# wusize/CLIPSelf

Hardware: AMD Instinct MI355X
Metric: images/sec (student+teacher distill step), ViT-B/16 32 crops/img (higher is better)
Workload: dtype bf16; 1 GPU; EVA02-CLIP-B-16 CLIPSelf image-patches step, 64 images x 32 crops per GPU, 224^2 (BASELINE configs[1]); global_batch=64, crops_per_image=32, image_size=224, parallelism=dp1, teacher_chunk=2048, teacher_last_block=cls_query_only, teacher_schedule=one_batch_ahead_on_side_stream

## Files before the change

clipself_amd/csrc/gemm_stream.hip:

```cpp
#include <vector>
#include <cstdio>
#include "gemm_common.h"

namespace {

typedef __attribute__((ext_vector_type(2))) unsigned u32x2;
typedef __attribute__((ext_vector_type(4))) unsigned u32x4;

constexpr unsigned OOB = 0xfffffff0u;

__device__ __forceinline__ float lane_bcast(int src_lane_x4, float v) {
    return __int_as_float(__builtin_amdgcn_ds_bpermute(src_lane_x4, __float_as_int(v)));
}
__device__ __forceinline__ unsigned pack2(float a, float b) {
    union { bf16x2 v; unsigned u; } pk;
    pk.v[0] = f2bf(a);
    pk.v[1] = f2bf(b);
    return pk.u;
}
__device__ __forceinline__ void swap32(unsigned& x, unsigned& y) {
    const u32x2 r = __builtin_amdgcn_permlane32_swap(x, y, false, false);
    x = r[0];
    y = r[1];
}
// ... 356 lines not shown

template <bool LN, bool AUX, int CP>
__device__ __forceinline__ void epi_swiglu_slab(const GemmArgs& p, const f32x16 (&acc)[4][2], int lane, int row0, int tn, int wn, const EpiOps& eo,
                                                char* slab) {
    const int l31 = lane & 31, hf = lane >> 5;
    const int hbase = tn * 128 + wn * 32;
    const bool colok = hbase < p.group;
    float nm[4], rs[4];
#pragma unroll
    for (int i = 0; i < 4; ++i) {
        rs[i] = LN ? eo.rstd[i] : 1.f;
        nm[i] = LN ? -eo.rstd[i] * eo.mean[i] : 0.f;
    }
    float ssum[4] = {0.f, 0.f, 0.f, 0.f}, ssq[4] = {0.f, 0.f, 0.f, 0.f};
    const int sl0 = hf << 4;
#pragma unroll
    for (int q = 0; q < 4; ++q) {
        float hv[4][4];
#pragma unroll
        for (int r = 0; r < 4; ++r) {
            const int e = q * 4 + r;
            const int sl = sl0 + ((8 * q + r) << 2);
            const float b1 = lane_bcast(sl, eo.cb), b2 = lane_bcast(sl + 128, eo.cb);
            float c1 = 0.f, c2 = 0.f;
            if (LN) { c1 = lane_bcast(sl, eo.cc); c2 = lane_bcast(sl + 128, eo.cc); }
#pragma unroll
            for (int i = 0; i < 4; ++i) {
                float u = acc[i][0][e], v = acc[i][1][e];
                if (LN) {
                    u = fmaf(rs[i], u, fmaf(nm[i], c1, b1));
                    v = fmaf(rs[i], v, fmaf(nm[i], c2, b2));
                } else {
                    u += b1;
                    v += b2;
                }
                hv[i][r] = silu_mul(u, v);
            }
        }
#pragma unroll
        for (int i = 0; i < 4; ++i) {
            const unsigned d0 = pack2(hv[i][0], hv[i][1]), d1 = pack2(hv[i][2], hv[i][3]);
            if (AUX) {
                ssum[i] = dot2_bf16(d1, 0x3f803f80u, dot2_bf16(d0, 0x3f803f80u, ssum[i]));
                ssq[i] = dot2_bf16(d1, d1, dot2_bf16(d0, d0, ssq[i]));
            }
            const int lrow = i * 32 + l31;
            const int s8 = (2 * q + hf) ^ (((lrow >> 1) & 3) << 1);
            *(uint2*)(slab + lrow * 64 + s8 * 8) = make_uint2(d0, d1);
        }
    }
    const __amdgpu_buffer_rsrc_t rc = make_rsrc((const __bf16*)p.C + (size_t)row0 * p.ldc + hbase);
    const int piece = lane & 3;
#pragma unroll
    for (int k = 0; k < 8; ++k) {
        const int lrow = (lane >> 2) + 16 * k;
        const uint4 w = *(const uint4*)(slab + lrow * 64 + ((piece ^ ((lrow >> 1) & 3)) << 4));
        const bool ok = colok && row0 + lrow < p.M && !CS_ABL(p, 8);
        store16<CP>(u32x4{w.x, w.y, w.z, w.w}, rc, ok ? (unsigned)(lrow * p.ldc + piece * 8) * 2u : OOB);
    }
    if (AUX) {
        const size_t slice = (size_t)tn * 4 + wn;
        const __amdgpu_buffer_rsrc_t rst = make_rsrc(p.stats_part + (slice * p.M + row0) * 2);
#pragma unroll
        for (int i = 0; i < 4; ++i) {
            const float s = both_halves(ssum[i]), q2 = both_halves(ssq[i]);
            const bool ok = colok && hf == 0 && row0 + i * 32 + l31 < p.M && !CS_ABL(p, 8);
            store8<CP>(u32x2{__float_as_uint(s), __float_as_uint(q2)}, rst, ok ? (unsigned)(i * 32 + l31) * 8u : OOB);
        }
    }
}

#ifdef CS_ABLATION_SWITCHES
__device__ unsigned long long* g_epi_trace = nullptr;
#define EPI_TRACE(slot)                                                                                                            \
    do {                                                                                                                           \
        if (g_epi_trace && (threadIdx.x & 63) == 0)                                                                                \
            g_epi_trace[((size_t)blockIdx.x * 8 + (threadIdx.x >> 6)) * 16 + (slot)] = __builtin_amdgcn_s_memrealtime();           \
    } while (0)
#define EPI_TRACE_WAIT() do { if (g_epi_trace) asm volatile("s_waitcnt vmcnt(0)" ::: "memory"); } while (0)
#else
#define EPI_TRACE(slot) do { } while (0)
#define EPI_TRACE_WAIT() do { } while (0)
#endif
template <bool LN, bool AUX, int CP, bool F8 = false, int SPLIT = 0, int FM = 4>
__device__ __forceinline__ void epi_resid_slab(const GemmArgs& p, const f32x16 (&acc)[FM][2], int lane, int row0, int colw, int tn, int wn,
                                               const EpiOps& eo, char* slab) {
    static_assert(!(SPLIT & 2) || AUX, "a split stream leaves together with the row statistics");
    const int l31 = lane & 31, hf = lane >> 5;
    const int rrow = lane >> 3, piece = lane & 7, col = colw + piece * 8;
    const bool colok = col < p.N;
    const __amdgpu_buffer_rsrc_t rc = make_rsrc((SPLIT & 2) ? (const void*)p.xb_out : (const void*)((const float*)p.C + (size_t)row0 * p.ldc + colw));
    const __amdgpu_buffer_rsrc_t rx = make_rsrc((SPLIT & 1) ? (const void*)p.xb_out : (const void*)(p.extra + (size_t)row0 * p.ldc + colw));
    const __amdgpu_buffer_rsrc_t rb = make_rsrc((AUX || SPLIT) ? (const void*)(p.xb_out + (size_t)row0 * p.ldxb + colw) : (const void*)p.C);
    const __amdgpu_buffer_rsrc_t rl = make_rsrc(SPLIT ? (const void*)(p.lo + (size_t)row0 * p.ldxb + colw) : (const void*)p.A);
    const size_t slice = (size_t)tn * 4 + wn;
    const __amdgpu_buffer_rsrc_t rst = make_rsrc(AUX ? (const void*)(p.stats_part + (slice * p.M + row0) * 2) : (const void*)p.C);
    f32x4 cb4[2] = {{0.f, 0.f, 0.f, 0.f}, {0.f, 0.f, 0.f, 0.f}}, cc4[2] = {{0.f, 0.f, 0.f, 0.f}, {0.f, 0.f, 0.f, 0.f}};
#pragma unroll
    for (int h = 0; h < 2; ++h) {
        const unsigned off = colok ? (unsigned)(col + 4 * h) * 4u : OOB;
        if (p.bias) cb4[h] = __builtin_bit_cast(f32x4, __builtin_amdgcn_raw_buffer_load_b128(make_rsrc(p.bias), off, 0, 0));
        if (LN || F8) cc4[h] = __builtin_bit_cast(f32x4, __builtin_amdgcn_raw_buffer_load_b128(make_rsrc(p.ln_colsum), off, 0, 0));
    }
    EPI_TRACE(0);
#pragma unroll
    for (int i = 0; i < FM; ++i) {
        f32x4 xin[4][2];
#pragma unroll
        for (int it = 0; it < 4; ++it) {
            const int rrel = i * 32 + rrow + 8 * it;
            const bool ok = colok && row0 + rrel < p.M;
            if constexpr (SPLIT & 1) {
                const unsigned off = ok ? (unsigned)(rrel * p.ldxb + piece * 8) * 2u : OOB;
                const u32x4 h = __builtin_bit_cast(u32x4, __builtin_amdgcn_raw_buffer_load_b128(rb, off, 0, CP));
                const u32x4 l = __builtin_bit_cast(u32x4, __builtin_amdgcn_raw_buffer_load_b128(rl, off, 0, CP));
#pragma unroll
                for (int w = 0; w < 4; ++w) {
                    xin[it][w >> 1][2 * (w & 1)] = __uint_as_float(__builtin_amdgcn_perm(h[w], l[w], 0x05040100u) - 0x8000u);
                    xin[it][w >> 1][2 * (w & 1) + 1] = __uint_as_float(__builtin_amdgcn_perm(h[w], l[w], 0x07060302u) - 0x8000u);
                }
            } else {
                const unsigned off = ok ? (unsigned)(rrel * p.ldc + piece * 8) * 4u : OOB;
                xin[it][0] = __builtin_bit_cast(f32x4, __builtin_amdgcn_raw_buffer_load_b128(rx, off, 0, CP));
                xin[it][1] = __builtin_bit_cast(f32x4, __builtin_amdgcn_raw_buffer_load_b128(rx, ok ? off + 16u : OOB, 0, CP));
            }
        }
        const float rs_row = (LN || F8) ? eo.rstd[i] : 1.f, nm_row = LN ? -eo.rstd[i] * eo.mean[i] : 0.f;
#pragma unroll
        for (int j = 0; j < 2; ++j)
#pragma unroll
            for (int q = 0; q < 4; ++q) {
                f32x4 t;
#pragma unroll
                for (int r = 0; r < 4; ++r) t[r] = acc[i][j][q * 4 + r];
                const int s16 = (j * 8 + 2 * q + hf) ^ (l31 & 15);
                *(f32x4*)(slab + l31 * 256 + s16 * 16) = t;
            }
        EPI_TRACE(1 + 3 * i);
        EPI_TRACE_WAIT();
        EPI_TRACE(2 + 3 * i);
        const int sel = lane & 7;
        float st_s = 0.f, st_q = 0.f;
#pragma unroll
        for (int it = 0; it < 4; ++it) {
            const int lrow = rrow + 8 * it, rrel = i * 32 + lrow;
            const bool ok = colok && row0 + rrel < p.M;
            float rs = 1.f, nm = 0.f;
            if (LN || F8) rs = lane_bcast(lrow << 2, rs_row);
            if (LN) nm = lane_bcast(lrow << 2, nm_row);
            f32x4 o[2];
#pragma unroll
            for (int h = 0; h < 2; ++h) {
                const f32x4 sv = *(const f32x4*)(slab + lrow * 256 + (((2 * piece + h) ^ (lrow & 15)) << 4));
                if (LN) {
#pragma unroll
                    for (int t = 0; t < 4; ++t) o[h][t] = xin[it][h][t] + fmaf(rs, sv[t], fmaf(nm, cc4[h][t], cb4[h][t]));
                } else if (F8) {
#pragma unroll
                    for (int t = 0; t < 4; ++t) o[h][t] = xin[it][h][t] + fmaf(rs * cc4[h][t], sv[t], cb4[h][t]);
                } else {
                    o[h] = xin[it][h] + (sv + cb4[h]);
                }
            }
            if constexpr (SPLIT & 2) {
                const unsigned off = ok ? (unsigned)(rrel * p.ldxb + piece * 8) * 2u : OOB;
                unsigned y[8];
#pragma unroll
                for (int t = 0; t < 8; ++t) y[t] = __float_as_uint(o[t >> 2][t & 3]) + 0x8000u;
                store16<CP>(u32x4{__builtin_amdgcn_perm(y[1], y[0], 0x07060302u), __builtin_amdgcn_perm(y[3], y[2], 0x07060302u),
                                  __builtin_amdgcn_perm(y[5], y[4], 0x07060302u), __builtin_amdgcn_perm(y[7], y[6], 0x07060302u)}, rb, off);
                store16<CP>(u32x4{__builtin_amdgcn_perm(y[1], y[0], 0x05040100u), __builtin_amdgcn_perm(y[3], y[2], 0x05040100u),
                                  __builtin_amdgcn_perm(y[5], y[4], 0x05040100u), __builtin_amdgcn_perm(y[7], y[6], 0x05040100u)}, rl, off);
            } else {
                const unsigned off = ok ? (unsigned)(rrel * p.ldc + piece * 8) * 4u : OOB;
                store16<CP>(__builtin_bit_cast(u32x4, o[0]), rc, off);
                store16<CP>(__builtin_bit_cast(u32x4, o[1]), rc, ok ? off + 16u : OOB);
            }
            if (AUX) {
                if constexpr (!(SPLIT & 2))
                    store16<CP>(u32x4{pack2(o[0][0], o[0][1]), pack2(o[0][2], o[0][3]), pack2(o[1][0], o[1][1]), pack2(o[1][2], o[1][3])}, rb,
                                ok ? (unsigned)(rrel * p.ldxb + piece * 8) * 2u : OOB);
                float ps = 0.f, pq = 0.f;
                if (colok) {
#pragma unroll
                    for (int t = 0; t < 8; ++t) { ps += o[t >> 2][t & 3]; pq = fmaf(o[t >> 2][t & 3], o[t >> 2][t & 3], pq); }
                }
                const float a = sum_lanes8(ps), b = sum_lanes8(pq);
                if (sel == it) { st_s = a; st_q = b; }
            }
        }
        if (AUX) {
            const int rrel = i * 32 + rrow + 8 * sel;
            const bool ok = sel < 4 && row0 + rrel < p.M && colw < p.N;
            store8<CP>(u32x2{__float_as_uint(st_s), __float_as_uint(st_q)}, rst, ok ? (unsigned)rrel * 8u : OOB);
        }
        EPI_TRACE(3 + 3 * i);
        __builtin_amdgcn_sched_barrier(0);
    }
}

template <int EPI, bool AUX, bool SLAB, int SPLIT = 0, int FM = 4, int MF = 32>
constexpr int epi_stores() {
    if (EPI == EPI_SWIGLU_BF16 && MF == 16) return 8 + (AUX ? 2 : 0);
    if (EPI == EPI_SWIGLU_BF16) return FM * (2 + (AUX ? 1 : 0));
    if (EPI == EPI_RESID_F32) return FM * (8 + (AUX ? ((SPLIT & 2) ? 0 : 4) + 1 : 0));
    return FM * 4;
}

#ifndef CS_DMA_AUX_A
#define CS_DMA_AUX_A 0
#endif
#ifndef CS_DMA_AUX_B
#define CS_DMA_AUX_B 0
#endif
#define CS_VMCNT(N) asm volatile("s_waitcnt vmcnt(%0)" ::"n"(N) : "memory")

inline bool getenv_flag(const char* name) {
    const char* v = getenv(name);
    return v && v[0] && v[0] != '0';
}

template <int EPI, bool LN, bool AUX, bool SLAB, bool F8 = false, int SPLIT = 0, int BMT = 256, int MF = 32>
__global__ __launch_bounds__(512) void gemm_stream_kernel(GemmArgs p) {
    static_assert(MF == 32 || (MF == 16 && LN && !SLAB && !F8 && SPLIT == 0 && BMT == 256 && (epi_is_bf16(EPI) ? !AUX : EPI == EPI_SWIGLU_BF16)),
                  "16x16x32 loop: the folded-LN bf16 and SwiGLU register epilogues");
    constexpr bool M16 = MF == 16;
    static_assert(BMT == 256 || (BMT == 192 && !F8 && SPLIT == 0 && !LN && !AUX), "192-row tiles: the training schedule's plain epilogues");
    static_assert(SPLIT == 0 || (EPI == EPI_RESID_F32 && LN && !F8), "the split stream belongs to the folded-LayerNorm residual epilogue");
    static_assert(SLAB || EPI != EPI_RESID_F32, "the fp32 residual epilogue exists in the slab form only (whole-line traffic)");
    static_assert(!F8 || (!LN && !AUX && (EPI == EPI_BF16 || EPI == EPI_RESID_F32)), "fp8 operands: bf16 and fp32-residual outputs");
    constexpr int ES = F8 ? 1 : 2;
    constexpr int CP = 0;
    constexpr bool SWI = EPI == EPI_SWIGLU_BF16, RES = EPI == EPI_RESID_F32;
    static_assert(SWI || RES || epi_is_bf16(EPI), "register epilogues");
    constexpr int BM = BMT, BN = 256, WN = 4, TM = BM / 2, TN = 64, FM = TM / 32, FN = 2;
    constexpr int A_BYTES = BM * BK * 2, B_BYTES = BN * BK * 2;
    constexpr int NPA = BM / 32;
    constexpr int NM = FM * FN, NR = FM + FN;
    constexpr int S = epi_stores<EPI, AUX, SLAB, SPLIT, FM, MF>() < 55 ? epi_stores<EPI, AUX, SLAB, SPLIT, FM, MF>() : 55;
    extern __shared__ __attribute__((aligned(16))) char smem[];
    const int tid = threadIdx.x, lane = tid & 63;
    const int wave = __builtin_amdgcn_readfirstlane(tid >> 6);
    const int wm = wave / WN, wn = wave - wm * WN;
    const int hf = M16 ? lane >> 4 : lane >> 5, l31 = M16 ? lane & 15 : lane & 31;
    char* const b_ring = smem + 3 * A_BYTES;
    const int ntiles = p.tiles_m * p.tiles_n, ktiles = p.K / (F8 ? 128 : BK);
    const int a_base = ((wm * TM + l31) >> 1) << 8, b_base = ((wn * TN + l31) >> 1) << 8;
    const int par8 = (l31 & 1) << 3, sw = l31 >> 1;
    const int G = gridDim.x;
#ifndef CS_NO_DMA_ROLES
    constexpr bool ROLES = !F8;
#else
    constexpr bool ROLES = false;
#endif
    const bool role_a = ROLES && wave >= 4;
#ifndef CS_NO_MID_BARRIER
    constexpr bool MID = ROLES && !SLAB && !F8;
#else
    constexpr bool MID = false;
#endif

    unsigned avoff[ROLES ? 8 : 4], bvoff[ROLES ? 1 : 4];
    const char *a_src = nullptr, *b_src = nullptr;
    int a_tile = blockIdx.x, a_kt = 0, b_tile = blockIdx.x, b_kt = 0;
    auto set_a = [&](int tile) {
        int tm, tn;
        tile_of_id(p, tile, ntiles, tm, tn);
        a_src = (const char*)p.A + (size_t)tm * BM * p.lda * ES;
#pragma unroll
        for (int i = 0; i < (ROLES ? NPA : 4); ++i) {
            int tr, chk;
            lane_source(ROLES ? (wave & 3) * NPA + i : wave * 4 + i, lane, tr, chk);
            avoff[i] = (unsigned)(min(tr, p.M - 1 - tm * BM) * p.lda * ES + chk * 16);
        }
    };
    auto set_b = [&](int tile) {
        int tm, tn;
        tile_of_id(p, tile, ntiles, tm, tn);
        if (SWI) {
            b_src = (const char*)p.B + (size_t)tn * (BN / 2) * p.ldb * ES;
        } else {
            b_src = (const char*)p.B + (size_t)tn * BN * p.ldb * ES;
        }
#pragma unroll
        for (int i = 0; i < (ROLES ? 8 : 4); ++i) {
            int tr, chk;
            lane_source(ROLES ? (wave & 3) * 8 + i : wave * 4 + i, lane, tr, chk);
            int rel;
            if (SWI) {
                const int hrel = (tr >> 6) * 32 + (tr & 31);
                rel = ((tr >> 5) & 1) * p.group + min(hrel, p.group - 1 - tn * (BN / 2));
            } else {
                rel = min(tr, p.N - 1 - tn * BN);
            }
            (ROLES ? avoff : bvoff)[i] = (unsigned)(rel * p.ldb * ES + chk * 16);
        }
    };
    auto adv_a = [&]() {
        if (++a_kt == ktiles) {
            a_kt = 0;
            if (a_tile + G < ntiles) {
                a_tile += G;
                set_a(a_tile);
            }
        }
    };
    auto adv_b = [&]() {
        if (++b_kt == ktiles) {
            b_kt = 0;
            if (b_tile + G < ntiles) {
                b_tile += G;
                set_b(b_tile);
            }
        }
    };
#define ISSUE_A(X, SLOT)                                                                                                      \
    __builtin_amdgcn_global_load_lds((const __attribute__((address_space(1))) void*)(a_src + (size_t)a_kt * (BK * 2) + avoff[X]), \
                                     (__attribute__((address_space(3))) void*)(smem + (SLOT) * A_BYTES + (wave * 4 + (X)) * 1024), 16, 0, CS_DMA_AUX_A)
#define ISSUE_B(X, SLOT)                                                                                                      \
    __builtin_amdgcn_global_load_lds((const __attribute__((address_space(1))) void*)(b_src + (size_t)b_kt * (BK * 2) + bvoff[X]), \
                                     (__attribute__((address_space(3))) void*)(b_ring + (SLOT) * B_BYTES + (wave * 4 + (X)) * 1024), 16, 0, CS_DMA_AUX_B)

#define ISSUE_RA(X, SLOT)                                                                                                     \
    __builtin_amdgcn_global_load_lds((const __attribute__((address_space(1))) void*)(a_src + (size_t)a_kt * (BK * 2) + avoff[X]), \
                                     (__attribute__((address_space(3))) void*)(smem + (SLOT) * A_BYTES + ((wave & 3) * NPA + (X)) * 1024), 16, 0, CS_DMA_AUX_A)
#define ISSUE_RB(X, SLOT)                                                                                                     \
    __builtin_amdgcn_global_load_lds((const __attribute__((address_space(1))) void*)(b_src + (size_t)b_kt * (BK * 2) + avoff[X]), \
                                     (__attribute__((address_space(3))) void*)(b_ring + (SLOT) * B_BYTES + ((wave & 3) * 8 + (X)) * 1024), 16, 0, CS_DMA_AUX_B)

    if constexpr (ROLES) {
        if (role_a) {
            set_a(a_tile);
#pragma unroll
            for (int x = 0; x < NPA; ++x) ISSUE_RA(x, 0);
            adv_a();
#pragma unroll
            for (int x = 0; x < NPA; ++x) ISSUE_RA(x, 1);
            adv_a();
        } else {
            set_b(b_tile);
#pragma unroll
            for (int x = 0; x < 8; ++x) ISSUE_RB(x, 0);
            adv_b();
            if constexpr (MID) {
#pragma unroll
                for (int x = 0; x < 8; ++x) ISSUE_RB(x, 1);
                adv_b();
            }
        }
        if constexpr (MID) {
            if (role_a) CS_VMCNT(NPA);
            else CS_VMCNT(8);
            __builtin_amdgcn_s_barrier();
        }
    } else {
        set_a(a_tile);
        set_b(b_tile);
#pragma unroll
        for (int x = 0; x < 4; ++x) ISSUE_A(x, 0);
        adv_a();
#pragma unroll
        for (int x = 0; x < 4; ++x) ISSUE_B(x, 0);
        adv_b();
#pragma unroll
        for (int x = 0; x < 4; ++x) ISSUE_A(x, 1);
        adv_a();
    }

    int curA = 0, gpar = 0;
    bool after_epi = false;
    for (int tile = blockIdx.x; tile < ntiles; tile += G) {
        int tm, tn;
        tile_of_id(p, tile, ntiles, tm, tn);
        const int row0 = tm * BM + wm * TM, colw = tn * BN + wn * TN;
        f32x16 acc[M16 ? 1 : FM][M16 ? 1 : FN];
        f32x4 acc16[M16 ? 8 : 1][M16 ? 4 : 1];
        constexpr int RB = M16 ? 16 : 32, NRB = TM / RB;
        EpiOpsT<M16 ? 8 : 4> eo;
        auto load_epi_ops = [&](int ln) {
            const int l31 = ln & (RB - 1), hf = ln >> 5, lane = ln;
#pragma unroll
            for (int i = 0; i < (M16 ? 8 : 4); ++i) eo.mean[i] = eo.rstd[i] = 0.f;
            eo.cb = eo.cc = 0.f;
            if (LN || F8) {
#pragma unroll
                for (int i = 0; i < NRB; ++i) {
                    const int r = min(row0 + i * RB + l31, p.M - 1);
                    if (LN) eo.mean[i] = p.ln_mean[r];
                    eo.rstd[i] = p.ln_rstd[r];
                }
            }
            int co;
            if (SWI) co = hf * p.group + min(tn * 128 + wn * 32 + (lane & 31), p.group - 1);
            else co = min(colw + lane, p.N - 1);
            if (!RES) {
                if (p.bias) eo.cb = p.bias[co];
                if (LN || F8) eo.cc = p.ln_colsum[co];
            }
        };

        auto ktile = [&](auto zero_tag, auto role_tag) {
            constexpr bool ZERO = decltype(zero_tag)::value;
            constexpr int ROLE = decltype(role_tag)::value;
            constexpr int KEEP = ROLE == 0 ? 4 : ROLE == 1 ? 0 : NPA;
            constexpr int SS = S + KEEP > 63 ? 63 - KEEP : S;
            if (after_epi) CS_VMCNT(KEEP + SS);
            else CS_VMCNT(KEEP);
            after_epi = false;
            asm volatile("s_waitcnt lgkmcnt(0)" ::: "memory");
            if (!CS_ABL(p, 2))
                __builtin_amdgcn_s_barrier();
            const char* la = smem + curA * A_BYTES + a_base;
            const char* lb = b_ring + gpar * B_BYTES + b_base;
            const int slot_a2 = curA == 0 ? 2 : curA - 1, slot_b1 = gpar ^ 1;
            if constexpr (F8) {
                typedef __attribute__((ext_vector_type(8))) int i32x8;
                typedef __attribute__((ext_vector_type(4))) int i32x4;
#pragma unroll
                for (int s2 = 0; s2 < 2; ++s2) {
                    const int c0 = 4 * s2 + 2 * hf;
                    const int off0 = ((par8 | c0) ^ sw) << 4, off1 = ((par8 | (c0 + 1)) ^ sw) << 4;
                    i32x8 a8[FM], b8[FN];
#pragma unroll
                    for (int i = 0; i < FM; ++i) {
                        const i32x4 lo = *(const i32x4*)(la + i * (16 * 256) + off0), hi = *(const i32x4*)(la + i * (16 * 256) + off1);
                        a8[i] = i32x8{lo[0], lo[1], lo[2], lo[3], hi[0], hi[1], hi[2], hi[3]};
                    }
#pragma unroll
                    for (int j = 0; j < FN; ++j) {
                        const i32x4 lo = *(const i32x4*)(lb + j * (16 * 256) + off0), hi = *(const i32x4*)(lb + j * (16 * 256) + off1);
                        b8[j] = i32x8{lo[0], lo[1], lo[2], lo[3], hi[0], hi[1], hi[2], hi[3]};
                    }
                    if constexpr (ROLE == 1) {
                        if (s2 == 0) {
#pragma unroll
                            for (int x = 0; x < 8; ++x) ISSUE_RB(x, slot_b1);
                        }
                    } else if constexpr (ROLE == 2) {
                        if (s2 == 1) {
#pragma unroll
                            for (int x = 0; x < NPA; ++x) ISSUE_RA(x, slot_a2);
                        }
                    } else if (s2 == 0) {
                        ISSUE_B(0, slot_b1); ISSUE_B(1, slot_b1); ISSUE_B(2, slot_b1); ISSUE_B(3, slot_b1);
                    } else {
                        ISSUE_A(0, slot_a2); ISSUE_A(1, slot_a2); ISSUE_A(2, slot_a2); ISSUE_A(3, slot_a2);
                    }
#pragma unroll
                    for (int i = 0; i < FM; ++i)
#pragma unroll
                        for (int j = 0; j < FN; ++j) {
                            if (ZERO && s2 == 0) {
                                const f32x16 z = {0.f, 0.f, 0.f, 0.f, 0.f, 0.f, 0.f, 0.f, 0.f, 0.f, 0.f, 0.f, 0.f, 0.f, 0.f, 0.f};
                                acc[i][j] = __builtin_amdgcn_mfma_scale_f32_32x32x64_f8f6f4(b8[j], a8[i], z, 0, 0, 0, 0x7f7f7f7f, 0, 0x7f7f7f7f);
                            } else {
                                acc[i][j] = __builtin_amdgcn_mfma_scale_f32_32x32x64_f8f6f4(b8[j], a8[i], acc[i][j], 0, 0, 0, 0x7f7f7f7f, 0, 0x7f7f7f7f);
                            }
                        }
                }
            } else {
                bf16x8 a[2][FM], b[2][FN];
                auto frags = [&](int ks, int buf) {
                    const int off = ((par8 | (ks * 2 + hf)) ^ sw) << 4;
#pragma unroll
                    for (int i = 0; i < FM; ++i) a[buf][i] = *(const bf16x8*)(la + i * (16 * 256) + off);
// ... 168 lines not shown
            };
            auto read_a = [&](const char* pa, int ks, int c) {
#pragma unroll
                for (int x = 0; x < 4; ++x) ga[c][x] = frag(pa, ks, c * 4 + x);
            };
            auto read_b = [&](const char* pb, int ks, int jj) {
                gb[2 * jj] = frag(pb, ks, 2 * jj);
                gb[2 * jj + 1] = frag(pb, ks, 2 * jj + 1);
            };
            auto mfmas = [&](int c, int jj, bool zero) {
#pragma unroll
                for (int x = 0; x < 4; ++x)
#pragma unroll
                    for (int j = 2 * jj; j < 2 * jj + 2; ++j) {
                        if (zero) {
                            const f32x4 z = {0.f, 0.f, 0.f, 0.f};
                            acc16[c * 4 + x][j] = __builtin_amdgcn_mfma_f32_16x16x32_bf16(gb[j], ga[c][x], z, 0, 0, 0);
                        } else {
                            acc16[c * 4 + x][j] = __builtin_amdgcn_mfma_f32_16x16x32_bf16(gb[j], ga[c][x], acc16[c * 4 + x][j], 0, 0, 0);
                        }
                    }
            };
            auto order = [&](auto r0a, auto nra, auto r0b, auto nrb, auto d0a, auto nda, auto d0b, auto ndb) {
#pragma unroll
                for (int m = 0; m < 16; ++m) {
                    __builtin_amdgcn_sched_group_barrier(0x008, 1, 0);
                    if ((m >= r0a.value && m < r0a.value + nra.value) || (m >= r0b.value && m < r0b.value + nrb.value))
                        __builtin_amdgcn_sched_group_barrier(0x100, 1, 0);
                    if ((m >= d0a.value && m < d0a.value + nda.value) || (m >= d0b.value && m < d0b.value + ndb.value))
                        __builtin_amdgcn_sched_group_barrier(0x010, 1, 0);
                }
            };
#define CI(N) std::integral_constant<int, (N)>{}
            if (ZERO) {
                read_a(la, 0, 0);
                read_b(lb, 0, 0);
                __builtin_amdgcn_sched_group_barrier(0x100, 6, 0);
            }
            read_b(lb, 0, 1);
            mfmas(0, 0, ZERO);
            read_a(la, 0, 1);
            mfmas(0, 1, ZERO);
            order(CI(0), CI(2), CI(8), CI(4), CI(0), CI(0), CI(0), CI(0));
            read_a(la, 1, 0);
            mfmas(1, 0, ZERO);
            read_b(lb, 1, 0);
            if constexpr (ROLE == 2) {
#pragma unroll
                for (int x = 0; x < NPA / 2; ++x) ISSUE_RA(x, slot_a2);
            }
            mfmas(1, 1, ZERO);
            order(CI(0), CI(4), CI(8), CI(2), CI(10), CI(ROLE == 2 ? NPA / 2 : 0), CI(0), CI(0));
            read_b(lb, 1, 1);
            if constexpr (ROLE == 2) {
#pragma unroll
                for (int x = NPA / 2; x < NPA; ++x) ISSUE_RA(x, slot_a2);
            }
            mfmas(0, 0, false);
            read_a(la, 1, 1);
            mfmas(0, 1, false);
            order(CI(0), CI(2), CI(8), CI(4), CI(2), CI(ROLE == 2 ? NPA / 2 : 0), CI(0), CI(0));
            {
                constexpr int KEEP = ROLE == 1 ? 0 : NPA;
                constexpr int SS = S + KEEP > 63 ? 63 - KEEP : S;
                if (after_epi) CS_VMCNT(KEEP + SS);
                else CS_VMCNT(KEEP);
                after_epi = false;
                asm volatile("s_waitcnt lgkmcnt(0)" ::: "memory");
                __builtin_amdgcn_s_barrier();
            }
            read_a(la_n, 0, 0);
            if constexpr (ROLE == 1) { ISSUE_RB(0, slot_b2); ISSUE_RB(1, slot_b2); ISSUE_RB(2, slot_b2); ISSUE_RB(3, slot_b2); }
            mfmas(1, 0, false);
            read_b(lb_n, 0, 0);
            if constexpr (ROLE == 1) { ISSUE_RB(4, slot_b2); ISSUE_RB(5, slot_b2); ISSUE_RB(6, slot_b2); ISSUE_RB(7, slot_b2); }
            mfmas(1, 1, false);
            order(CI(0), CI(4), CI(8), CI(2), CI(4), CI(ROLE == 1 ? 4 : 0), CI(10), CI(ROLE == 1 ? 4 : 0));
#undef CI
            if (ROLE == 1) adv_b();
            else adv_a();
            curA = nextA;
            gpar ^= 1;
        };
        if constexpr (M16) {
            if (role_a) {
                ktile_m16(std::true_type{}, std::integral_constant<int, 2>{});
                for (int kt = 1; kt < ktiles; ++kt) ktile_m16(std::false_type{}, std::integral_constant<int, 2>{});
            } else {
                ktile_m16(std::true_type{}, std::integral_constant<int, 1>{});
                for (int kt = 1; kt < ktiles; ++kt) ktile_m16(std::false_type{}, std::integral_constant<int, 1>{});
            }
        } else if constexpr (MID) {
            if (role_a) {
                ktile_mid(std::true_type{}, std::integral_constant<int, 2>{});
                for (int kt = 1; kt < ktiles; ++kt) ktile_mid(std::false_type{}, std::integral_constant<int, 2>{});
            } else {
                ktile_mid(std::true_type{}, std::integral_constant<int, 1>{});
                for (int kt = 1; kt < ktiles; ++kt) ktile_mid(std::false_type{}, std::integral_constant<int, 1>{});
            }
        } else if constexpr (ROLES) {
            if (role_a) {
                ktile(std::true_type{}, std::integral_constant<int, 2>{});
                for (int kt = 1; kt < ktiles; ++kt) ktile(std::false_type{}, std::integral_constant<int, 2>{});
            } else {
                ktile(std::true_type{}, std::integral_constant<int, 1>{});
                for (int kt = 1; kt < ktiles; ++kt) ktile(std::false_type{}, std::integral_constant<int, 1>{});
            }
        } else {
            ktile(std::true_type{}, std::integral_constant<int, 0>{});
            for (int kt = 1; kt < ktiles; ++kt) ktile(std::false_type{}, std::integral_constant<int, 0>{});
        }
        if (CS_ABL(p, 4)) continue;
        after_epi = true;
        int lane_e = lane;
        asm volatile("" : "+v"(lane_e));
        if constexpr (SLAB) {
            asm volatile("s_waitcnt lgkmcnt(0)" ::: "memory");
            __builtin_amdgcn_s_barrier();
            char* const slab = wave >= 4 ? b_ring + (gpar ^ 1) * B_BYTES + (wave - 4) * 8192
                               : (BM == 192 && wave == 3) ? b_ring + 2 * B_BYTES
                                                          : smem + (curA == 0 ? 2 : curA - 1) * A_BYTES + wave * 8192;
            load_epi_ops(lane_e);
#ifndef CS_NO_KERNARG_RELOAD
            constexpr bool RELOAD = RES && LN && AUX;
#else
            constexpr bool RELOAD = false;
#endif
            if constexpr (RELOAD) {
                const __attribute__((address_space(4))) GemmArgs* pk = (const __attribute__((address_space(4))) GemmArgs*)__builtin_amdgcn_kernarg_segment_ptr();
                asm volatile("" : "+s"(pk));
                GemmArgs pe;
                pe.A = pk->A; pe.C = pk->C; pe.bias = pk->bias; pe.extra = pk->extra; pe.M = pk->M; pe.N = pk->N; pe.ldc = pk->ldc;
                pe.ln_colsum = pk->ln_colsum; pe.stats_part = pk->stats_part; pe.xb_out = pk->xb_out; pe.ldxb = pk->ldxb; pe.lo = pk->lo;
                pe.dbg = pk->dbg;
                epi_resid_slab<LN, AUX, CP, F8, SPLIT, FM>(pe, acc, lane_e, row0, colw, tn, wn, eo, slab);
            } else if constexpr (RES) {
                epi_resid_slab<LN, AUX, CP, F8, SPLIT, FM>(p, acc, lane_e, row0, colw, tn, wn, eo, slab);
            } else {
                static_assert(FM == 4, "the slab forms of the bf16 / SwiGLU epilogues exist for 256-row tiles");
                if constexpr (SWI) epi_swiglu_slab<LN, AUX, CP>(p, acc, lane_e, row0, tn, wn, eo, slab);
                else epi_bf16_slab<epi_act(EPI), LN, CP>(p, acc, lane_e, row0, colw, eo, slab);
            }
        } else {
            load_epi_ops(lane_e);
            if constexpr (M16 && SWI) epi_swiglu_m16<LN, AUX, CP>(p, acc16, lane_e, row0, tn, wn, eo);
            else if constexpr (M16) epi_bf16_m16<epi_act(EPI), LN, CP>(p, acc16, lane_e, row0, colw, eo);
            else if constexpr (SWI) epi_swiglu<LN, AUX, CP, FM>(p, acc, lane_e, row0, tn, wn, eo);
            else epi_bf16<epi_act(EPI), LN, CP, F8, FM>(p, acc, lane_e, row0, colw, eo);
        }
    }
    CS_VMCNT(0);
#undef ISSUE_A
#undef ISSUE_B
#undef ISSUE_RA
#undef ISSUE_RB
}

template <int EPI, bool LN, bool AUX, bool SLAB, int BMT = 256, int MF = 32>
int launch_stream_v(const GemmArgs& a, unsigned grid, hipStream_t stream) {
    constexpr size_t lds = 160 * 1024;
    static bool once = ((void)hipFuncSetAttribute((const void*)gemm_stream_kernel<EPI, LN, AUX, SLAB, false, 0, BMT, MF>, hipFuncAttributeMaxDynamicSharedMemorySize, (int)lds), true);
    (void)once;
    hipLaunchKernelGGL((gemm_stream_kernel<EPI, LN, AUX, SLAB, false, 0, BMT, MF>), dim3(grid), dim3(512), lds, stream, a);
    CS_LAUNCH_CHECK();
    return 0;
}

template <int EPI, bool LN, bool AUX>
int launch_stream_t(const GemmArgs& a, unsigned grid, hipStream_t stream) {
    if constexpr (EPI == EPI_RESID_F32) return launch_stream_v<EPI, LN, AUX, true>(a, grid, stream);
    else if (a.dbg & 1) return launch_stream_v<EPI, LN, AUX, true>(a, grid, stream);
    else if constexpr (LN && (epi_is_bf16(EPI) ? !AUX : EPI == EPI_SWIGLU_BF16)) {
        if (!getenv_flag("CS_GEMM_MFMA32")) return launch_stream_v<EPI, LN, AUX, false, 256, 16>(a, grid, stream);
        return launch_stream_v<EPI, LN, AUX, false>(a, grid, stream);
    } else return launch_stream_v<EPI, LN, AUX, false>(a, grid, stream);
}

template <bool AUX, int SPLIT>
int launch_stream_split(const GemmArgs& a, unsigned grid, hipStream_t stream) {
    constexpr size_t lds = 160 * 1024;
    static bool once = ((void)hipFuncSetAttribute((const void*)gemm_stream_kernel<EPI_RESID_F32, true, AUX, true, false, SPLIT>,
                                                  hipFuncAttributeMaxDynamicSharedMemorySize, (int)lds), true);
    (void)once;
    hipLaunchKernelGGL((gemm_stream_kernel<EPI_RESID_F32, true, AUX, true, false, SPLIT>), dim3(grid), dim3(512), lds, stream, a);
    CS_LAUNCH_CHECK();
    return 0;
}

template <int EPI>
int launch_stream_bf16(const GemmArgs& a, unsigned grid, hipStream_t stream) {
    return a.ln_mean ? launch_stream_t<EPI, true, false>(a, grid, stream) : launch_stream_t<EPI, false, false>(a, grid, stream);
}

template <int EPI, bool SLAB>
int launch_stream_f8(const GemmArgs& a, unsigned grid, hipStream_t stream) {
    constexpr size_t lds = 160 * 1024;
    static bool once = ((void)hipFuncSetAttribute((const void*)gemm_stream_kernel<EPI, false, false, SLAB, true>, hipFuncAttributeMaxDynamicSharedMemorySize, (int)lds), true);
    (void)once;
    hipLaunchKernelGGL((gemm_stream_kernel<EPI, false, false, SLAB, true>), dim3(grid), dim3(512), lds, stream, a);
    CS_LAUNCH_CHECK();
    return 0;
}

}

int cs_gemm_stream_launch_f8(GemmArgs a, int epi, int reserve, hipStream_t stream) {
    a.tiles_m = (a.M + 255) / 256;
    a.tiles_n = (a.N + 255) / 256;
    const long ntiles = (long)a.tiles_m * a.tiles_n;
    const long cap = cs_persistent_cap(reserve);
    const unsigned grid = (unsigned)(ntiles < cap ? ntiles : cap);
    if (epi == EPI_BF16) return launch_stream_f8<EPI_BF16, false>(a, grid, stream);
    return launch_stream_f8<EPI_RESID_F32, true>(a, grid, stream);
}

#ifdef CS_ABLATION_SWITCHES
static int stream_launch_impl(GemmArgs a, int epi, int reserve, hipStream_t stream);
int cs_gemm_stream_launch(GemmArgs a, int epi, int reserve, hipStream_t stream) {
    static const char* path = getenv("CS_GEMM_TRACE");
    static unsigned long long* buf = nullptr;
    constexpr size_t WORDS = 256 * 8 * 16;
    if (path && !buf && hipMalloc((void**)&buf, WORDS * 8) == hipSuccess) {
        (void)hipMemset(buf, 0, WORDS * 8);
        (void)hipMemcpyToSymbol(HIP_SYMBOL(g_epi_trace), &buf, sizeof(buf));
    }
    const int rc = stream_launch_impl(a, epi, reserve, stream);
    if (path && buf && rc == 0 && (epi == EPI_RESID_F32 || epi == EPI_RESID_LN_F32)) {
        (void)hipStreamSynchronize(stream);
        std::vector<unsigned long long> host(WORDS);
        (void)hipMemcpy(host.data(), buf, WORDS * 8, hipMemcpyDeviceToHost);
        if (FILE* f = fopen(path, "wb")) { fwrite(host.data(), 8, WORDS, f); fclose(f); }
    }
    return rc;
}
static int stream_launch_impl(GemmArgs a, int epi, int reserve, hipStream_t stream) {
#else
int cs_gemm_stream_launch(GemmArgs a, int epi, int reserve, hipStream_t stream) {
#endif
    const bool swi = epi == EPI_SWIGLU_BF16, res = epi == EPI_RESID_F32 || epi == EPI_RESID_LN_F32;
    if (!(swi || res || epi == EPI_BF16 || epi == EPI_QGELU_BF16)) return 1;
    if (a.M < 1 || a.K % BK != 0) return 1;
    if (swi ? (a.group % 32 != 0) : (a.N % 32 != 0)) return 1;
    if ((long)a.ldc * 128 * 4 >= 0x70000000L || (long)a.ldxb * 128 * 2 >= 0x70000000L) return 1;
    const bool ln = a.ln_mean != nullptr;
    if ((epi == EPI_RESID_LN_F32) != (res && ln)) return 1;
    bool aux = false;
    if (swi) aux = a.stats_part != nullptr;
    else if (res) {
        if ((a.stats_part != nullptr) != (a.xb_out != nullptr)) return 1;
        aux = a.stats_part != nullptr;
        if (aux && (a.ldxb % 8 != 0 || ((uintptr_t)a.xb_out % 16) != 0)) return 1;
    } else if (a.stats_part || a.xb_out) return 1;
    a.tiles_m = (a.M + 255) / 256;
    a.tiles_n = swi ? (a.group + 127) / 128 : (a.N + 255) / 256;
    long ntiles = (long)a.tiles_m * a.tiles_n;
    const long cap = cs_persistent_cap(reserve);
    unsigned grid = (unsigned)(ntiles < cap ? ntiles : cap);
    if (!ln && !aux && !(a.dbg & 1) && a.M >= 192 && (swi || res || epi == EPI_BF16) && !getenv_flag("CS_NO_BM192")) {
        const long t192 = (long)((a.M + 191) / 192) * a.tiles_n;
        const long c256 = ((ntiles + cap - 1) / cap) * 256, c192 = ((t192 + cap - 1) / cap) * 192;
        if (c192 * 10 < c256 * 9) {
            a.tiles_m = (a.M + 191) / 192;
            ntiles = t192;
            grid = (unsigned)(ntiles < cap ? ntiles : cap);
            if (swi) return launch_stream_v<EPI_SWIGLU_BF16, false, false, false, 192>(a, grid, stream);
            if (res) return launch_stream_v<EPI_RESID_F32, false, false, true, 192>(a, grid, stream);
            return launch_stream_v<EPI_BF16, false, false, false, 192>(a, grid, stream);
        }
    }
// ... 67 lines not shown
```

Before: 760.1 images/sec.

## Route folded-LN residual GEMMs through 16x16x32 MFMA main loop by default

Extends the 16x16x32 bf16 MFMA main loop to the slab-based folded-LayerNorm fp32 residual epilogue and its split-stream variants. It adds a new scheduled k-tile body (ktile_t16) for the non-mid-role case and a 16x16 accumulator-to-slab scatter in the residual epilogue. The default launch now selects this path, with an environment variable to fall back to the 32x32 loop. It aims to improve MFMA throughput and scheduling for these GEMMs, at the cost of more accumulator registers, different LDS fragment reads, and a new hand-ordered schedule that may or may not beat the old one.

```diff
diff --git a/clipself_amd/csrc/gemm_stream.hip b/clipself_amd/csrc/gemm_stream.hip
--- a/clipself_amd/csrc/gemm_stream.hip
+++ b/clipself_amd/csrc/gemm_stream.hip
@@ -462,11 +462,14 @@
 #define EPI_TRACE(slot) do { } while (0)
 #define EPI_TRACE_WAIT() do { } while (0)
 #endif
-template <bool LN, bool AUX, int CP, bool F8 = false, int SPLIT = 0, int FM = 4>
-__device__ __forceinline__ void epi_resid_slab(const GemmArgs& p, const f32x16 (&acc)[FM][2], int lane, int row0, int colw, int tn, int wn,
+template <bool LN, bool AUX, int CP, bool F8 = false, int SPLIT = 0, int FM = 4, int MF = 32, typename ACC>
+__device__ __forceinline__ void epi_resid_slab(const GemmArgs& p, const ACC& acc, int lane, int row0, int colw, int tn, int wn,
                                                const EpiOps& eo, char* slab) {
     static_assert(!(SPLIT & 2) || AUX, "a split stream leaves together with the row statistics");
+    static_assert(MF == 32 || (MF == 16 && FM == 4 && !F8), "16x16 accumulator blocks: 256-row tiles, bf16 operands");
+    constexpr bool M16 = MF == 16;
     const int l31 = lane & 31, hf = lane >> 5;
+    const int l15 = lane & 15, g16 = lane >> 4;
     const int rrow = lane >> 3, piece = lane & 7, col = colw + piece * 8;
     const bool colok = col < p.N;
     const __amdgpu_buffer_rsrc_t rc = make_rsrc((SPLIT & 2) ? (const void*)p.xb_out : (const void*)((const float*)p.C + (size_t)row0 * p.ldc + colw));
@@ -506,16 +509,23 @@
             }
         }
         const float rs_row = (LN || F8) ? eo.rstd[i] : 1.f, nm_row = LN ? -eo.rstd[i] * eo.mean[i] : 0.f;
-#pragma unroll
-        for (int j = 0; j < 2; ++j)
-#pragma unroll
-            for (int q = 0; q < 4; ++q) {
-                f32x4 t;
-#pragma unroll
-                for (int r = 0; r < 4; ++r) t[r] = acc[i][j][q * 4 + r];
-                const int s16 = (j * 8 + 2 * q + hf) ^ (l31 & 15);
-                *(f32x4*)(slab + l31 * 256 + s16 * 16) = t;
-            }
+        if constexpr (M16) {
+#pragma unroll
+            for (int b = 0; b < 2; ++b)
+#pragma unroll
+                for (int j = 0; j < 4; ++j) *(f32x4*)(slab + (16 * b + l15) * 256 + (((4 * j + g16) ^ l15) << 4)) = acc[2 * i + b][j];
+        } else {
+#pragma unroll
+            for (int j = 0; j < 2; ++j)
+#pragma unroll
+                for (int q = 0; q < 4; ++q) {
+                    f32x4 t;
+#pragma unroll
+                    for (int r = 0; r < 4; ++r) t[r] = acc[i][j][q * 4 + r];
+                    const int s16 = (j * 8 + 2 * q + hf) ^ (l31 & 15);
+                    *(f32x4*)(slab + l31 * 256 + s16 * 16) = t;
+                }
+        }
         EPI_TRACE(1 + 3 * i);
         EPI_TRACE_WAIT();
         EPI_TRACE(2 + 3 * i);
@@ -602,8 +612,9 @@
 
 template <int EPI, bool LN, bool AUX, bool SLAB, bool F8 = false, int SPLIT = 0, int BMT = 256, int MF = 32>
 __global__ __launch_bounds__(512) void gemm_stream_kernel(GemmArgs p) {
-    static_assert(MF == 32 || (MF == 16 && LN && !SLAB && !F8 && SPLIT == 0 && BMT == 256 && (epi_is_bf16(EPI) ? !AUX : EPI == EPI_SWIGLU_BF16)),
-                  "16x16x32 loop: the folded-LN bf16 and SwiGLU register epilogues");
+    static_assert(MF == 32 || (MF == 16 && LN && !F8 && BMT == 256 &&
+                               (SLAB ? EPI == EPI_RESID_F32 : SPLIT == 0 && (epi_is_bf16(EPI) ? !AUX : EPI == EPI_SWIGLU_BF16))),
+                  "16x16x32 loop: the folded-LN bf16 and SwiGLU register epilogues, and the whole folded-LN residual family (fp32 and split streams)");
     constexpr bool M16 = MF == 16;
     static_assert(BMT == 256 || (BMT == 192 && !F8 && SPLIT == 0 && !LN && !AUX), "192-row tiles: the training schedule's plain epilogues");
     static_assert(SPLIT == 0 || (EPI == EPI_RESID_F32 && LN && !F8), "the split stream belongs to the folded-LayerNorm residual epilogue");
@@ -643,10 +654,16 @@
     unsigned avoff[ROLES ? 8 : 4], bvoff[ROLES ? 1 : 4];
     const char *a_src = nullptr, *b_src = nullptr;
     int a_tile = blockIdx.x, a_kt = 0, b_tile = blockIdx.x, b_kt = 0;
+    auto lane_of_cursor = [&]() {
+        int l = lane;
+        if constexpr (M16 && SLAB) asm volatile("" : "+v"(l));
+        return l;
+    };
     auto set_a = [&](int tile) {
         int tm, tn;
         tile_of_id(p, tile, ntiles, tm, tn);
         a_src = (const char*)p.A + (size_t)tm * BM * p.lda * ES;
+        const int lane = lane_of_cursor();
 #pragma unroll
         for (int i = 0; i < (ROLES ? NPA : 4); ++i) {
             int tr, chk;
@@ -662,6 +679,7 @@
         } else {
             b_src = (const char*)p.B + (size_t)tn * BN * p.ldb * ES;
         }
+        const int lane = lane_of_cursor();
 #pragma unroll
         for (int i = 0; i < (ROLES ? 8 : 4); ++i) {
             int tr, chk;
@@ -755,12 +773,12 @@
         const int row0 = tm * BM + wm * TM, colw = tn * BN + wn * TN;
         f32x16 acc[M16 ? 1 : FM][M16 ? 1 : FN];
         f32x4 acc16[M16 ? 8 : 1][M16 ? 4 : 1];
-        constexpr int RB = M16 ? 16 : 32, NRB = TM / RB;
-        EpiOpsT<M16 ? 8 : 4> eo;
+        constexpr int RB = M16 && !RES ? 16 : 32, NRB = TM / RB;
+        EpiOpsT<RB == 16 ? 8 : 4> eo;
         auto load_epi_ops = [&](int ln) {
             const int l31 = ln & (RB - 1), hf = ln >> 5, lane = ln;
 #pragma unroll
-            for (int i = 0; i < (M16 ? 8 : 4); ++i) eo.mean[i] = eo.rstd[i] = 0.f;
+            for (int i = 0; i < (RB == 16 ? 8 : 4); ++i) eo.mean[i] = eo.rstd[i] = 0.f;
             eo.cb = eo.cc = 0.f;
             if (LN || F8) {
 #pragma unroll
@@ -1095,7 +1113,115 @@
             curA = nextA;
             gpar ^= 1;
         };
-        if constexpr (M16) {
+        auto ktile_t16 = [&](auto zero_tag, auto role_tag) {
+            constexpr bool ZERO = decltype(zero_tag)::value;
+            constexpr int ROLE = decltype(role_tag)::value;
+            constexpr int KEEP = ROLE == 0 ? 4 : ROLE == 1 ? 0 : NPA;
+            constexpr int SS = S + KEEP > 63 ? 63 - KEEP : S;
+            if (after_epi) CS_VMCNT(KEEP + SS);
+            else CS_VMCNT(KEEP);
+            after_epi = false;
+            asm volatile("s_waitcnt lgkmcnt(0)" ::: "memory");
+            if (!CS_ABL(p, 2))
+                __builtin_amdgcn_s_barrier();
+            const char* la = smem + curA * A_BYTES + a_base;
+            const char* lb = b_ring + gpar * B_BYTES + b_base;
+            const int slot_a2 = curA == 0 ? 2 : curA - 1, slot_b1 = gpar ^ 1;
+            bf16x8 ha[2][4], hb[4];
+            auto frag = [&](const char* base, int ks, int blk) {
+                const int off = (((par8 | (ks * 4 + hf)) ^ sw) << 4) ^ ((blk & 1) << 7);
+                return *(const bf16x8*)(base + blk * (8 * 256) + off);
+            };
+            auto read_a = [&](int ks, int c) {
+#pragma unroll
+                for (int x = 0; x < 4; ++x) ha[c][x] = frag(la, ks, c * 4 + x);
+            };
+            auto read_b = [&](int ks, int jj) {
+                hb[2 * jj] = frag(lb, ks, 2 * jj);
+                hb[2 * jj + 1] = frag(lb, ks, 2 * jj + 1);
+            };
+            auto mfmas = [&](int c, int jj, bool zero) {
+#pragma unroll
+                for (int x = 0; x < 4; ++x)
+#pragma unroll
+                    for (int j = 2 * jj; j < 2 * jj + 2; ++j) {
+                        if (zero) {
+                            const f32x4 z = {0.f, 0.f, 0.f, 0.f};
+                            acc16[c * 4 + x][j] = __builtin_amdgcn_mfma_f32_16x16x32_bf16(hb[j], ha[c][x], z, 0, 0, 0);
+                        } else {
+                            acc16[c * 4 + x][j] = __builtin_amdgcn_mfma_f32_16x16x32_bf16(hb[j], ha[c][x], acc16[c * 4 + x][j], 0, 0, 0);
+                        }
+                    }
+            };
+            auto order = [&](auto r0a, auto nra, auto r0b, auto nrb, auto d0, auto nd) {
+#ifndef CS_NO_SGB
+#pragma unroll
+                for (int m = 0; m < 16; ++m) {
+                    __builtin_amdgcn_sched_group_barrier(0x008, 1, 0);
+                    if ((m >= r0a.value && m < r0a.value + nra.value) || (m >= r0b.value && m < r0b.value + nrb.value))
+                        __builtin_amdgcn_sched_group_barrier(0x100, 1, 0);
+                    if (m >= d0.value && m < d0.value + nd.value) __builtin_amdgcn_sched_group_barrier(0x010, 1, 0);
+                }
+#endif
+            };
+#define CI(N) std::integral_constant<int, (N)>{}
+            constexpr int NB1 = ROLE == 1 ? 4 : ROLE == 0 ? 2 : 0;
+            constexpr int NA2 = ROLE == 2 ? NPA / 2 : ROLE == 0 ? 2 : 0;
+            read_a(0, 0);
+            read_b(0, 0);
+#ifndef CS_NO_SGB
+            __builtin_amdgcn_sched_group_barrier(0x100, 6, 0);
+#endif
+            read_b(0, 1);
+            mfmas(0, 0, ZERO);
+            read_a(0, 1);
+            if constexpr (ROLE == 1) { ISSUE_RB(0, slot_b1); ISSUE_RB(1, slot_b1); ISSUE_RB(2, slot_b1); ISSUE_RB(3, slot_b1); }
+            if constexpr (ROLE == 0) { ISSUE_B(0, slot_b1); ISSUE_B(1, slot_b1); }
+            mfmas(0, 1, ZERO);
+            order(CI(0), CI(2), CI(8), CI(4), CI(12), CI(NB1));
+            read_a(1, 0);
+            mfmas(1, 0, ZERO);
+            read_b(1, 0);
+            if constexpr (ROLE == 1) { ISSUE_RB(4, slot_b1); ISSUE_RB(5, slot_b1); ISSUE_RB(6, slot_b1); ISSUE_RB(7, slot_b1); }
+            if constexpr (ROLE == 0) { ISSUE_B(2, slot_b1); ISSUE_B(3, slot_b1); }
+            mfmas(1, 1, ZERO);
+            order(CI(0), CI(4), CI(8), CI(2), CI(10), CI(NB1));
+            read_b(1, 1);
+            mfmas(0, 0, false);
+            read_a(1, 1);
+            if constexpr (ROLE == 2) {
+#pragma unroll
+                for (int x = 0; x < NPA / 2; ++x) ISSUE_RA(x, slot_a2);
+            }
+            if constexpr (ROLE == 0) { ISSUE_A(0, slot_a2); ISSUE_A(1, slot_a2); }
+            mfmas(0, 1, false);
+            order(CI(0), CI(2), CI(8), CI(4), CI(12), CI(NA2));
+            if constexpr (ROLE == 2) {
+#pragma unroll
+                for (int x = NPA / 2; x < NPA; ++x) ISSUE_RA(x, slot_a2);
+            }
+            if constexpr (ROLE == 0) { ISSUE_A(2, slot_a2); ISSUE_A(3, slot_a2); }
+            mfmas(1, 0, false);
+            mfmas(1, 1, false);
+            order(CI(0), CI(0), CI(0), CI(0), CI(2), CI(NA2));
+#undef CI
+            if (ROLE != 2) adv_b();
+            if (ROLE != 1) adv_a();
+            curA = curA == 2 ? 0 : curA + 1;
+            gpar ^= 1;
+        };
+        if constexpr (M16 && !MID) {
+            if constexpr (!ROLES) {
+                ktile_t16(std::true_type{}, std::integral_constant<int, 0>{});
+                for (int kt = 1; kt < ktiles; ++kt) ktile_t16(std::false_type{}, std::integral_constant<int, 0>{});
+            } else if (role_a) {
+                ktile_t16(std::true_type{}, std::integral_constant<int, 2>{});
+                for (int kt = 1; kt < ktiles; ++kt) ktile_t16(std::false_type{}, std::integral_constant<int, 2>{});
+            } else {
+                ktile_t16(std::true_type{}, std::integral_constant<int, 1>{});
+                for (int kt = 1; kt < ktiles; ++kt) ktile_t16(std::false_type{}, std::integral_constant<int, 1>{});
+            }
+        } else if constexpr (M16) {
             if (role_a) {
                 ktile_m16(std::true_type{}, std::integral_constant<int, 2>{});
                 for (int kt = 1; kt < ktiles; ++kt) ktile_m16(std::false_type{}, std::integral_constant<int, 2>{});
@@ -1146,9 +1272,11 @@
                 pe.A = pk->A; pe.C = pk->C; pe.bias = pk->bias; pe.extra = pk->extra; pe.M = pk->M; pe.N = pk->N; pe.ldc = pk->ldc;
                 pe.ln_colsum = pk->ln_colsum; pe.stats_part = pk->stats_part; pe.xb_out = pk->xb_out; pe.ldxb = pk->ldxb; pe.lo = pk->lo;
                 pe.dbg = pk->dbg;
-                epi_resid_slab<LN, AUX, CP, F8, SPLIT, FM>(pe, acc, lane_e, row0, colw, tn, wn, eo, slab);
+                if constexpr (M16) epi_resid_slab<LN, AUX, CP, F8, SPLIT, FM, 16>(pe, acc16, lane_e, row0, colw, tn, wn, eo, slab);
+                else epi_resid_slab<LN, AUX, CP, F8, SPLIT, FM>(pe, acc, lane_e, row0, colw, tn, wn, eo, slab);
             } else if constexpr (RES) {
-                epi_resid_slab<LN, AUX, CP, F8, SPLIT, FM>(p, acc, lane_e, row0, colw, tn, wn, eo, slab);
+                if constexpr (M16) epi_resid_slab<LN, AUX, CP, F8, SPLIT, FM, 16>(p, acc16, lane_e, row0, colw, tn, wn, eo, slab);
+                else epi_resid_slab<LN, AUX, CP, F8, SPLIT, FM>(p, acc, lane_e, row0, colw, tn, wn, eo, slab);
             } else {
                 static_assert(FM == 4, "the slab forms of the bf16 / SwiGLU epilogues exist for 256-row tiles");
                 if constexpr (SWI) epi_swiglu_slab<LN, AUX, CP>(p, acc, lane_e, row0, tn, wn, eo, slab);
@@ -1181,7 +1309,10 @@
 
 template <int EPI, bool LN, bool AUX>
 int launch_stream_t(const GemmArgs& a, unsigned grid, hipStream_t stream) {
-    if constexpr (EPI == EPI_RESID_F32) return launch_stream_v<EPI, LN, AUX, true>(a, grid, stream);
+    if constexpr (EPI == EPI_RESID_F32 && LN) {
+        if (!getenv_flag("CS_GEMM_MFMA32")) return launch_stream_v<EPI, LN, AUX, true, 256, 16>(a, grid, stream);
+        return launch_stream_v<EPI, LN, AUX, true>(a, grid, stream);
+    } else if constexpr (EPI == EPI_RESID_F32) return launch_stream_v<EPI, LN, AUX, true>(a, grid, stream);
     else if (a.dbg & 1) return launch_stream_v<EPI, LN, AUX, true>(a, grid, stream);
     else if constexpr (LN && (epi_is_bf16(EPI) ? !AUX : EPI == EPI_SWIGLU_BF16)) {
         if (!getenv_flag("CS_GEMM_MFMA32")) return launch_stream_v<EPI, LN, AUX, false, 256, 16>(a, grid, stream);
@@ -1189,15 +1320,20 @@
     } else return launch_stream_v<EPI, LN, AUX, false>(a, grid, stream);
 }
 
+template <bool AUX, int SPLIT, int MF>
+int launch_stream_split_v(const GemmArgs& a, unsigned grid, hipStream_t stream) {
+    constexpr size_t lds = 160 * 1024;
+    static bool once = ((void)hipFuncSetAttribute((const void*)gemm_stream_kernel<EPI_RESID_F32, true, AUX, true, false, SPLIT, 256, MF>,
+                                                  hipFuncAttributeMaxDynamicSharedMemorySize, (int)lds), true);
+    (void)once;
+    hipLaunchKernelGGL((gemm_stream_kernel<EPI_RESID_F32, true, AUX, true, false, SPLIT, 256, MF>), dim3(grid), dim3(512), lds, stream, a);
+    CS_LAUNCH_CHECK();
+    return 0;
+}
 template <bool AUX, int SPLIT>
 int launch_stream_split(const GemmArgs& a, unsigned grid, hipStream_t stream) {
-    constexpr size_t lds = 160 * 1024;
-    static bool once = ((void)hipFuncSetAttribute((const void*)gemm_stream_kernel<EPI_RESID_F32, true, AUX, true, false, SPLIT>,
-                                                  hipFuncAttributeMaxDynamicSharedMemorySize, (int)lds), true);
-    (void)once;
-    hipLaunchKernelGGL((gemm_stream_kernel<EPI_RESID_F32, true, AUX, true, false, SPLIT>), dim3(grid), dim3(512), lds, stream, a);
-    CS_LAUNCH_CHECK();
-    return 0;
+    if (!getenv_flag("CS_GEMM_MFMA32")) return launch_stream_split_v<AUX, SPLIT, 16>(a, grid, stream);
+    return launch_stream_split_v<AUX, SPLIT, 32>(a, grid, stream);
 }
 
 template <int EPI>
```

Result: no change. 765.3 images/sec (median of 6 runs) (+0.7%).
